# kdu3613/Multimodal_GAR

Measured on AMD Instinct MI355X. Metric: clips/sec (fwd+bwd) at 32 actors x 16k pts x 15 frames, higher is better.
Workload: dtype f32; 1 GPU; c3: 8 clips x 15 frames x 32 actors x 16384 pts, 720x1280 RGB, fp32 fwd+bwd+Adam, LiDAR route pointnet2, GAT on; global_clips=8, clips_per_gpu=8, parallelism=dp1, launch=hip_graph, geometry=in step, gradient_exchange=none, trainable_params=29692332

## Files before the change

include/mgar_ops.h:

```cpp
#ifndef MGAR_OPS_H
#define MGAR_OPS_H

#ifdef __cplusplus
extern "C" {
#endif

#define MGAR_OK 0
#define MGAR_EINVAL (-1)
#define MGAR_ELAUNCH (-2)
#define MGAR_EUNSUPPORTED (-3)

#define MGAR_MAX_NSAMPLE 128
#define MGAR_ABI_VERSION 22

int mgar_abi_version(void);
const char *mgar_last_error(void);

int mgar_ktimer_enable(int on);
int mgar_ktimer_count(void);
const char *mgar_ktimer_name(int id);
int mgar_ktimer_read(int id, double *total_ms, long long *launches, double *total_bytes, double *total_flops,
                     int reset);
int mgar_ktimer_add_flops(int id, double flops);
int mgar_ktimer_add_bytes(int id, double bytes);
// ... 209 lines not shown
                                  int Cout, const float *in_mean, const float *in_invstd, const float *in_gamma,
                                  const float *in_beta, int in_relu, float *y, float *out_stats, void *stream);

int mgar_bn_act_maxpool_bwd_reduce(const float *dpool, long long sb, long long sc, long long sm, const float *pooled,
                                   const unsigned char *arg, const float *x, const float *xarg, int B, int C, int M,
                                   int nsample, const float *mean, const float *invstd, int relu, float *workspace,
                                   float *dgamma, float *dbeta, float *coef, float *dmask, void *stream);
int mgar_pointwise_conv_fwd_maxgrad(const float *x4, int B, int Cin, int M, int nsample, const float *w, int w_row_stride,
                                    int w_col_stride, int Cout, const float *mean, const float *invstd, const float *gamma,
                                    const float *coef, const unsigned char *arg, const float *dmask, float *y, void *stream);
int mgar_pointwise_conv_dw_maxgrad(const float *x, const float *x4, int B, int Cin, int Cout, int M, int nsample,
                                   const float *in_mean, const float *in_invstd, const float *in_gamma,
                                   const float *in_beta, int in_relu, const float *mean, const float *invstd,
                                   const float *gamma, const float *coef, const unsigned char *arg, const float *dmask,
                                   float *workspace, float *dw, void *stream);

int mgar_pointwise_conv_maxpool_eval_fwd(const float *x, int B, int Cin, int M, int nsample, const float *w,
                                         int w_row_stride, int w_col_stride, int Cout, const float *in_mean,
                                         const float *in_invstd, const float *in_gamma, const float *in_beta, int in_relu,
                                         const float *out_scale, const float *out_shift, int out_relu, float *pooled,
                                         void *stream);

int mgar_pointwise_mfma_bf16_fwd(const void *x, int B, int Cin, int P, const float *w, int w_row_stride, int w_col_stride,
                                 int Cout, const float *in_mean, const float *in_invstd, const float *in_gamma,
                                 const float *in_beta, int in_relu, void *y, void *stream);

int mgar_pointwise_wide_bf16_fwd(const void *x, int B, int Cin, int P, const float *w, int w_ld, int Cout,
                                 const float *in_mean, const float *in_invstd, const float *in_gamma, const float *in_beta,
                                 int in_relu, const float *out_scale, const float *out_shift, int out_relu, void *y,
                                 long long y_batch_stride, void *stream);
// ... 230 lines not shown
```

multimodal_gar_amd/bn_ops.py:

```python
import os

import torch
import torch.nn as nn
from torch.autograd import Function
from torch.autograd.function import once_differentiable

from . import _lib as L


def _u8ptr(t):
    return L.dev_ptr(t, torch.uint8)


def _workspace(x, b, c, p):
    return torch.empty((L.raw("mgar_bn_workspace_floats", b, c, p),), dtype=torch.float32, device=x.device)


_PAYLOADS = (torch.float32, torch.bfloat16)


def _f32(t):
    return t if t is None or t.dtype == torch.float32 else t.float()


# ... 130 lines not shown
        ctx.relu = relu
        return y

    @staticmethod
    @once_differentiable
    def backward(ctx, gy):
        x3, gamma, beta, mean, invstd, w = ctx.saved_tensors
        b, c, p = x3.shape
        cout = w.shape[0]
        gy = gy.contiguous()
        st = L.stream_of(x3)
        ga = torch.empty_like(x3)
        L.call("mgar_pointwise_conv_fwd", L.fptr(gy), b, cout, p, L.fptr(w), 1, c, c, None, None, None, None, 0,
               L.fptr(ga), st)
        dgamma, dbeta = torch.empty_like(gamma), torch.empty_like(gamma)
        if FUSED_DW_BN_REDUCE and ctx.needs_input_grad[6]:
            dw = torch.empty_like(w)
            coef = torch.empty((2 * c,), dtype=torch.float32, device=x3.device)
            wsd = torch.empty((max(1, L.raw("mgar_pointwise_dw_bnbwd_workspace_floats", b, c, cout, p)),), dtype=torch.float32,
                              device=x3.device)
            L.call("mgar_pointwise_conv_dw_bnbwd", L.fptr(x3), L.fptr(gy), L.fptr(w), b, c, cout, p, L.fptr(mean), L.fptr(invstd),
                   L.fptr(gamma), L.fptr(beta), int(ctx.relu), L.fptr(wsd), L.fptr(dw), L.fptr(dgamma), L.fptr(dbeta), L.fptr(coef), st)
            dx = torch.empty((b, p, c) if ctx.rowmajor else (b, c, p), dtype=torch.float32, device=x3.device)
            L.call("mgar_bn_act_bwd_apply", L.fptr(ga), L.fptr(x3), b, c, p, L.fptr(mean), L.fptr(invstd), L.fptr(gamma), L.fptr(beta),
                   int(ctx.relu), L.fptr(coef), int(ctx.rowmajor), L.fptr(dx), st)
            return (dx.permute(0, 2, 1) if ctx.rowmajor else dx), dgamma, dbeta, None, None, None, dw, None, None
        dw = None
        if ctx.needs_input_grad[6]:
            dw = torch.empty_like(w)
            wsd = torch.empty((max(1, L.raw("mgar_pointwise_dw_workspace_floats", b, c, cout, p)),), dtype=torch.float32,
                              device=x3.device)
# ... 47 lines not shown
        coef2 = torch.empty((2 * ck,), dtype=torch.float32, device=dev)
        dmask = torch.empty((b, ck, m), dtype=torch.float32, device=dev)
        ws2 = _workspace(x4, b, ck, p)
        if dpool.dtype == torch.float32 and dpool.dim() == 3 and not dpool.is_contiguous() \
                and (b == 1 or dpool.stride(0) >= 0) and min(dpool.stride(1), dpool.stride(2)) >= 1:
            dp, strides = dpool, (dpool.stride(0) if b > 1 else 0, dpool.stride(1), dpool.stride(2))
        else:
            dp, strides = dpool.contiguous().float(), (0, -1, 1)
        L.call("mgar_bn_act_maxpool_bwd_reduce", dp.data_ptr(), strides[0], strides[1], strides[2], L.fptr(out), _u8ptr(arg),
               L.fptr(x4), L.fptr(xarg) if xarg is not None else None, b, ck, m, ns, L.fptr(mean2), L.fptr(invstd2),
               int(ctx.relu2), L.fptr(ws2), L.fptr(dgamma2), L.fptr(dbeta2), L.fptr(coef2), L.fptr(dmask), st)
        ga = torch.empty_like(x3)
        L.call("mgar_pointwise_conv_fwd_maxgrad", L.fptr(x4), b, ck, m, ns, L.fptr(w), 1, c, c, L.fptr(mean2), L.fptr(invstd2),
               L.fptr(gamma2), L.fptr(coef2), _u8ptr(arg), L.fptr(dmask), L.fptr(ga), st)
        dw = None
        if ctx.needs_input_grad[6]:
            dw = torch.empty_like(w)
            wsd = torch.empty((max(1, L.raw("mgar_pointwise_dw_workspace_floats", b, c, ck, p)),), dtype=torch.float32, device=dev)
            L.call("mgar_pointwise_conv_dw_maxgrad", L.fptr(x3), L.fptr(x4), b, c, ck, m, ns, L.fptr(mean), L.fptr(invstd),
                   L.fptr(gamma), L.fptr(beta), int(ctx.relu), L.fptr(mean2), L.fptr(invstd2), L.fptr(gamma2), L.fptr(coef2),
                   _u8ptr(arg), L.fptr(dmask), L.fptr(wsd), L.fptr(dw), st)
        dgamma, dbeta = torch.empty_like(gamma), torch.empty_like(gamma)
        ws = _workspace(x3, b, c, p)
        if ctx.rowmajor:
            dx = _bwd_rowmajor(ga, x3, mean, invstd, gamma, beta, ctx.relu, ws, dgamma, dbeta)
        else:
            dx = torch.empty_like(x3)
            L.call("mgar_bn_act_bwd", L.fptr(ga), L.fptr(x3), b, c, p, L.fptr(mean), L.fptr(invstd), L.fptr(gamma),
                   L.fptr(beta), int(ctx.relu), L.fptr(ws), L.fptr(dgamma), L.fptr(dbeta), L.fptr(dx), st)
        return dx, dgamma, dbeta, None, None, None, dw, dgamma2, dbeta2, None, None, None, None, None


class _PlainConv(Function):

    @staticmethod
    def forward(ctx, x3, w, out_stats=None):
        b, c, p = x3.shape
# ... 41 lines not shown
        return None
    c, cout = x.shape[1], conv.out_channels
    x3 = x.contiguous().flatten(2)
    if c > PLAIN_CONV_MAX_IN or cout > PLAIN_CONV_MAX_OUT or x3.shape[2] % 4 != 0 or x3.shape[0] * x3.shape[2] < (1 << 16):
        return None
    needs_grad = torch.is_grad_enabled() and (x.requires_grad or conv.weight.requires_grad)
    if bf16_mfma and mlp_bf16_mfma_plan(x3, cout, needs_grad, None, PLAIN_CONV_MAX_IN, PLAIN_CONV_MAX_OUT):
        y = _conv_bf16_mfma(x3, _f32(conv.weight.detach()).view(cout, c), None, None, None, None, False)
        y = y.view(x.shape[0], cout, *x.shape[2:])
        return (y, None) if want_out_stats else y
    out_stats = stats_partial_buffer(x3, cout, x3.shape[0] * x3.shape[2]) if want_out_stats and x3.shape[2] % STATS_TILE == 0 else None
    y = _PlainConv.apply(x3, _f32(conv.weight).view(cout, c), out_stats).view(x.shape[0], cout, *x.shape[2:])
    return (y, out_stats) if want_out_stats else y


FUSED_DW_BN_REDUCE = False
FUSED_CONV_MAX_CHANNELS = 64


FUSED_STATS_MAX_CHANNELS = 32


MLP_BF16_MFMA = os.environ.get("MGAR_MLP_BF16_MFMA", "1") != "0"


def mlp_bf16_mfma_plan(x, cout, needs_grad, bn=None, max_in=FUSED_CONV_MAX_CHANNELS, max_out=FUSED_CONV_MAX_CHANNELS):
    if not (MLP_BF16_MFMA and x.dtype == torch.bfloat16 and x.is_cuda and len(x.shape) >= 3) or needs_grad:
        return False
    if bn is not None and not bn.training:
        return False
    c, p = x.shape[1], 1
# ... 504 lines not shown
```

multimodal_gar_amd/csrc/pointwise_dw.hip:

```cpp
#include "common.hpp"

namespace mgar {

typedef float __attribute__((ext_vector_type(16))) f32x16;

constexpr int DW_TP = 128;
constexpr int DW_LD = DW_TP + 1;

struct DwAct {
    const float *mean, *invstd, *gamma, *beta;
    int relu;
    int pair;
};

struct DwGrad {
    const float *mean, *invstd, *gamma;
    const float *coef;
    const unsigned char *arg;
    const float *d;
    int M, ns;
};

template <int OB, int IB, bool GRAD = false>
__global__ __launch_bounds__(256) void pointwise_dw_kernel(const float *__restrict__ x, const float *__restrict__ dy, int B, int Cin,
                                                           int Cout, int P, DwAct act, float *__restrict__ partial, DwGrad g) {
    extern __shared__ float lds[];
    constexpr int GR = GRAD ? OB * 32 : 1;
    __shared__ float g_k[GR], g_m0[GR], g_mu[GR], g_is[GR], g_m1[GR];
    __shared__ float act_sc[IB * 32], act_sh[IB * 32], act_mu[IB * 32];
    __shared__ float act_is[IB * 32];
    float *sy = lds;
    float *sx = lds + OB * 32 * DW_LD;
    const int o_base = blockIdx.y * OB * 32, i_base = blockIdx.z * IB * 32;
    const bool has_act = act.mean != nullptr;
    const bool pair = act.pair != 0;
    const int CinV = pair ? 2 * Cin : Cin;
    if constexpr (GRAD) {
        for (int r = threadIdx.x; r < OB * 32; r += 256) {
            const int ch = o_base + r;
            const bool ok = ch < Cout;
            const float is = ok ? g.invstd[ch] : 0.f;
            g_mu[r] = ok ? g.mean[ch] : 0.f;
            g_is[r] = is;
            g_k[r] = ok ? (g.gamma ? g.gamma[ch] : 1.f) * is : 0.f;
            g_m0[r] = ok ? g.coef[2 * ch] : 0.f;
            g_m1[r] = ok ? g.coef[2 * ch + 1] : 0.f;
        }
        if (!has_act) __syncthreads();
    }
    if (has_act) {
        for (int r = threadIdx.x; r < IB * 32; r += 256) {
            const int chv = i_base + r, ch = (pair && chv >= Cin) ? chv - Cin : chv;
            float sc = 1.f, sh = 0.f, mu = 0.f, is = 0.f;
            if (chv < CinV) {
                sc = act.invstd[ch] * (act.gamma ? act.gamma[ch] : 1.f);
                sh = act.beta ? act.beta[ch] : 0.f;
                mu = act.mean[ch];
                is = act.invstd[ch];
            }
            act_sc[r] = sc;
            act_sh[r] = sh;
            act_mu[r] = mu;
            act_is[r] = is;
        }
        __syncthreads();
    }
    auto pair_of = [&](float v, int r, bool kind) {
        const float mu = act_mu[r];
        const bool on = !act.relu || !((v - mu) * act_sc[r] + act_sh[r] <= 0.f);
        return on ? (kind ? (v - mu) * act_is[r] : 1.f) : 0.f;
    };
    const int lane = threadIdx.x & 63, wave = threadIdx.x >> 6;
    const int tiles_per_b = (P + DW_TP - 1) / DW_TP;
    const long long total_tiles = (long long)B * tiles_per_b;
    const bool vec = (P & 3) == 0;

    f32x16 acc[OB][IB];
#pragma unroll
    for (int a = 0; a < OB; ++a)
#pragma unroll
        for (int c = 0; c < IB; ++c)
#pragma unroll
            for (int r = 0; r < 16; ++r) acc[a][c][r] = 0.f;

    constexpr int NV = (OB + IB) * 32 * (DW_TP / 4) / 256;
    float4 pre[NV];
    constexpr int NG = GRAD ? OB * 4 : 1;
    float pre_d[NG];
    int pre_a[NG], pre_s0 = 0;
    auto fetch = [&](long long tile) {
        const int b = (int)(tile / tiles_per_b);
        const int p0 = (int)(tile - (long long)b * tiles_per_b) * DW_TP;
        if constexpr (GRAD) {
            const int p = p0 + (threadIdx.x & 31) * 4;
            const int m = (int)((unsigned)p / (unsigned)g.ns);
            pre_s0 = p - m * g.ns;
#pragma unroll
            for (int u = 0; u < NG; ++u) {
                const int ch = o_base + (threadIdx.x >> 5) + 8 * u;
                const bool ok = ch < Cout && p < P;
                const size_t go = ((size_t)b * Cout + ch) * g.M + m;
                pre_d[u] = ok ? g.d[go] : 0.f;
                pre_a[u] = ok ? (int)g.arg[go] : 0;
            }
        }
#pragma unroll
        for (int u = 0; u < NV; ++u) {
            const int e = threadIdx.x + u * 256;
            const int row = e / (DW_TP / 4), c4 = (e - row * (DW_TP / 4)) * 4;
            const bool is_y = row < OB * 32;
            const int chv = is_y ? o_base + row : i_base + row - OB * 32;
            const int ch = (!is_y && pair && chv >= Cin) ? chv - Cin : chv;
            const int cmax = is_y ? Cout : Cin;
            pre[u] = (chv < (is_y ? Cout : CinV) && p0 + c4 < P)
                         ? *reinterpret_cast<const float4 *>((is_y ? dy : x) + ((size_t)b * cmax + ch) * P + p0 + c4)
                         : make_float4(0.f, 0.f, 0.f, 0.f);
        }
    };
    if (vec && (long long)blockIdx.x < total_tiles) fetch(blockIdx.x);

    for (long long tile = blockIdx.x; tile < total_tiles; tile += gridDim.x) {
        const int b = (int)(tile / tiles_per_b);
        const int p0 = (int)(tile - (long long)b * tiles_per_b) * DW_TP;
        if (vec) {
#pragma unroll
            for (int u = 0; u < NV; ++u) {
                const int e = threadIdx.x + u * 256;
                const int row = e / (DW_TP / 4), c4 = (e - row * (DW_TP / 4)) * 4;
                const bool is_y = row < OB * 32;
                const int ch = is_y ? o_base + row : i_base + row - OB * 32;
                float4 v = pre[u];
                if constexpr (GRAD) {
                    if (u < NG && ch < Cout && p0 + c4 < P) {
                        const float k = g_k[row], m0 = g_m0[row], mu = g_mu[row], is = g_is[row], m1 = g_m1[row];
                        const float d = pre_d[u < NG ? u : 0];
                        const int sa = pre_a[u < NG ? u : 0] - pre_s0;
                        v.x = k * ((sa == 0 ? d : 0.f) - m0 - (v.x - mu) * is * m1);
                        v.y = k * ((sa == 1 ? d : 0.f) - m0 - (v.y - mu) * is * m1);
                        v.z = k * ((sa == 2 ? d : 0.f) - m0 - (v.z - mu) * is * m1);
                        v.w = k * ((sa == 3 ? d : 0.f) - m0 - (v.w - mu) * is * m1);
                    }
                }
                if (has_act && !is_y && ch < CinV && p0 + c4 < P) {
                    const int r = row - OB * 32;
                    if (pair) {
                        const bool kind = ch >= Cin;
                        v.x = pair_of(v.x, r, kind); v.y = pair_of(v.y, r, kind); v.z = pair_of(v.z, r, kind); v.w = pair_of(v.w, r, kind);
                    } else {
                        const float sc = act_sc[r], sh = act_sh[r], mu = act_mu[r];
                        v.x = (v.x - mu) * sc + sh; v.y = (v.y - mu) * sc + sh; v.z = (v.z - mu) * sc + sh; v.w = (v.w - mu) * sc + sh;
                        if (act.relu) { v.x = relu_nan(v.x); v.y = relu_nan(v.y); v.z = relu_nan(v.z); v.w = relu_nan(v.w); }
                    }
                }
                float *d = lds + row * DW_LD + c4;
                d[0] = v.x; d[1] = v.y; d[2] = v.z; d[3] = v.w;
            }
        } else {
            for (int e = threadIdx.x; e < (OB + IB) * 32 * DW_TP; e += 256) {
                const int row = e / DW_TP, cc = e - row * DW_TP;
                const bool is_y = row < OB * 32;
                const int chv = is_y ? o_base + row : i_base + row - OB * 32;
                const int ch = (!is_y && pair && chv >= Cin) ? chv - Cin : chv;
                const int cmax = is_y ? Cout : Cin;
                float v = 0.f;
                if (chv < (is_y ? Cout : CinV) && p0 + cc < P) {
                    v = (is_y ? dy : x)[((size_t)b * cmax + ch) * P + p0 + cc];
                    if (has_act && !is_y) {
                        if (pair) {
                            v = pair_of(v, row - OB * 32, chv >= Cin);
                        } else {
                            v = (v - act_mu[row - OB * 32]) * act_sc[row - OB * 32] + act_sh[row - OB * 32];
                            if (act.relu) v = relu_nan(v);
                        }
                    }
                }
                lds[row * DW_LD + cc] = v;
            }
        }
        __syncthreads();
        if (vec && tile + gridDim.x < total_tiles) fetch(tile + gridDim.x);
        const int colw = wave * 32 + (lane >> 5);
#pragma unroll 4
        for (int ks = 0; ks < 16; ++ks) {
            const int cc = colw + 2 * ks;
            float af[OB], bf[IB];
#pragma unroll
            for (int a = 0; a < OB; ++a) af[a] = sy[(a * 32 + (lane & 31)) * DW_LD + cc];
#pragma unroll
            for (int c = 0; c < IB; ++c) bf[c] = sx[(c * 32 + (lane & 31)) * DW_LD + cc];
#pragma unroll
            for (int a = 0; a < OB; ++a)
#pragma unroll
                for (int c = 0; c < IB; ++c)
                    acc[a][c] = __builtin_amdgcn_mfma_f32_32x32x2f32(af[a], bf[c], acc[a][c], 0, 0, 0);
        }
        __syncthreads();
    }
    if (wave > 0) {
#pragma unroll
        for (int a = 0; a < OB; ++a)
#pragma unroll
            for (int c = 0; c < IB; ++c)
#pragma unroll
                for (int r = 0; r < 16; ++r) lds[(((wave - 1) * OB * IB + a * IB + c) * 16 + r) * 64 + lane] = acc[a][c][r];
    }
    __syncthreads();
    if (wave > 0) return;
#pragma unroll
    for (int a = 0; a < OB; ++a)
#pragma unroll
        for (int c = 0; c < IB; ++c)
#pragma unroll
            for (int r = 0; r < 16; ++r) {
                float v = acc[a][c][r];
#pragma unroll
                for (int w = 0; w < 3; ++w) v += lds[((w * OB * IB + a * IB + c) * 16 + r) * 64 + lane];
                const int o = o_base + a * 32 + (r & 3) + 8 * (r >> 2) + 4 * (lane >> 5);
                const int i = i_base + c * 32 + (lane & 31);
                if (o < Cout && i < CinV) partial[((size_t)blockIdx.x * Cout + o) * CinV + i] = v;
            }
}

constexpr int DWR_SLICES = 16;
__global__ __launch_bounds__(64 * DWR_SLICES) void pointwise_dw_reduce_kernel(const float *__restrict__ partial, int gx, int n_out,
                                                                              float *__restrict__ dw) {
    __shared__ float part[DWR_SLICES][64];
    const int e = blockIdx.x * 64 + (threadIdx.x & 63), slice = threadIdx.x >> 6;
    const int per = (gx + DWR_SLICES - 1) / DWR_SLICES, g0 = min(slice * per, gx), g1 = min(g0 + per, gx);
    float s = 0.f;
    if (e < n_out) {
        int g = g0;
        for (; g + 8 <= g1; g += 8) {
            float v[8];
#pragma unroll
// ... 34 lines not shown
}

static int dw_grid_x(int B, int Cin, int Cout, int P, int ob, int ib) {
    const long long tiles = (long long)B * ((P + DW_TP - 1) / DW_TP);
    const int gy = ceil_div(Cout, ob * 32), gz = ceil_div(Cin, ib * 32);
    long long gx = 2048 / (gy * gz);
    if (gx > (tiles + 3) / 4) gx = (tiles + 3) / 4;
    if (gx < 1) gx = 1;
    return (int)gx;
}
static void dw_blocks(int Cin, int Cout, int &ob, int &ib) {
    ob = Cout <= 32 ? 1 : 2;
    ib = Cin <= 32 ? 1 : (Cin <= 64 ? 2 : 4);
}

template <int OB, int IB, bool GRAD = false>
static void launch_dw(const float *x, const float *dy, int B, int Cin, int Cout, int P, const DwAct &act, float *partial,
                      hipStream_t st, const DwGrad &g = DwGrad{}) {
    static bool attr_set = false;
    const int lds = (OB + IB) * 32 * DW_LD * (int)sizeof(float);
    if (!attr_set) {
        (void)hipFuncSetAttribute((const void *)pointwise_dw_kernel<OB, IB, GRAD>, hipFuncAttributeMaxDynamicSharedMemorySize, lds);
        attr_set = true;
    }
    const int CinV = act.pair ? 2 * Cin : Cin;
    const int gy = ceil_div(Cout, OB * 32), gz = ceil_div(CinV, IB * 32);
    const int gx = dw_grid_x(B, CinV, Cout, P, OB, IB);
    hipLaunchKernelGGL((pointwise_dw_kernel<OB, IB, GRAD>), dim3((unsigned)gx, gy, gz), dim3(256), lds, st, x, dy, B, Cin, Cout, P, act, partial, g);
}

}

using namespace mgar;

MGAR_API int mgar_pointwise_dw_workspace_floats(int B, int Cin, int Cout, int P) {
    if (B <= 0 || Cin <= 0 || Cout <= 0 || P <= 0) return 0;
    int ob, ib;
    dw_blocks(Cin, Cout, ob, ib);
    return dw_grid_x(B, Cin, Cout, P, ob, ib) * Cout * Cin;
}

MGAR_API int mgar_pointwise_conv_dw_act(const float *x, const float *dy, int B, int Cin,
                                        int Cout, int P, const float *in_mean,
// ... 1 lines not shown
                                        const float *in_beta, int in_relu,
                                        float *workspace, float *dw, void *stream) {
    MGAR_REQUIRE(B >= 0 && Cin >= 0 && Cout >= 0 && P >= 0, "pointwise_conv_dw: negative size");
    if (Cin == 0 || Cout == 0) return MGAR_OK;
    MGAR_REQUIRE(dw, "pointwise_conv_dw: null pointer");
    MGAR_REQUIRE(in_mean == nullptr || in_invstd != nullptr, "pointwise_conv_dw: in_mean without in_invstd");
    hipStream_t st = (hipStream_t)stream;
    if ((long long)B * P == 0) {
        (void)hipMemsetAsync(dw, 0, sizeof(float) * Cout * Cin, st);
        return check_launch("pointwise_conv_dw: memset failed");
    }
    MGAR_REQUIRE(x && dy && workspace, "pointwise_conv_dw: null pointer");
    const DwAct act{in_mean, in_invstd, in_gamma, in_beta, in_relu, 0};
    int ob, ib;
    dw_blocks(Cin, Cout, ob, ib);
    {
    KtScope kt(KT_POINTWISE_DW, st, 4.0 * (double)B * P * (Cin + Cout), 2.0 * (double)B * P * Cin * Cout);
    if (ob == 1 && ib == 1) launch_dw<1, 1>(x, dy, B, Cin, Cout, P, act, workspace, st);
    else if (ob == 1 && ib == 2) launch_dw<1, 2>(x, dy, B, Cin, Cout, P, act, workspace, st);
    else if (ob == 1 && ib == 4) launch_dw<1, 4>(x, dy, B, Cin, Cout, P, act, workspace, st);
    else if (ob == 2 && ib == 1) launch_dw<2, 1>(x, dy, B, Cin, Cout, P, act, workspace, st);
    else if (ob == 2 && ib == 2) launch_dw<2, 2>(x, dy, B, Cin, Cout, P, act, workspace, st);
    else launch_dw<2, 4>(x, dy, B, Cin, Cout, P, act, workspace, st);
    }
    const int gx = dw_grid_x(B, Cin, Cout, P, ob, ib), n_out = Cout * Cin;
    hipLaunchKernelGGL(pointwise_dw_reduce_kernel, dim3(ceil_div(n_out, 64)), dim3(64 * DWR_SLICES), 0, st, workspace, gx, n_out, dw);
    return check_launch("pointwise_conv_dw: launch failed");
}

MGAR_API int mgar_pointwise_conv_dw(const float *x, const float *dy, int B, int Cin,
                                    int Cout, int P, float *workspace, float *dw,
                                    void *stream) {
    return mgar_pointwise_conv_dw_act(x, dy, B, Cin, Cout, P, nullptr, nullptr, nullptr, nullptr, 0, workspace, dw, stream);
}

MGAR_API int mgar_pointwise_conv_dw_maxgrad(const float *x, const float *x4, int B, int Cin, int Cout, int M, int nsample,
                                            const float *in_mean, const float *in_invstd, const float *in_gamma,
                                            const float *in_beta, int in_relu, const float *mean, const float *invstd,
                                            const float *gamma, const float *coef, const unsigned char *arg, const float *dmask,
                                            float *workspace, float *dw, void *stream) {
// ... 6 lines not shown
        set_error("pointwise_conv_dw_maxgrad: needs Cin <= 64, Cout <= 64 and nsample % 4 == 0 (write the gradient with "
                  "mgar_bn_act_maxpool_bwd otherwise)");
        return MGAR_EUNSUPPORTED;
    }
    hipStream_t st = (hipStream_t)stream;
    if ((long long)B * M == 0) {
        (void)hipMemsetAsync(dw, 0, sizeof(float) * Cout * Cin, st);
        return check_launch("pointwise_conv_dw_maxgrad: memset failed");
    }
    MGAR_REQUIRE(x && x4 && workspace && mean && invstd && coef && arg && dmask, "pointwise_conv_dw_maxgrad: null pointer");
    const int P = M * nsample;
    const DwAct act{in_mean, in_invstd, in_gamma, in_beta, in_relu, 0};
    const DwGrad g{mean, invstd, gamma, coef, arg, dmask, M, nsample};
    int ob, ib;
    dw_blocks(Cin, Cout, ob, ib);
    {
    KtScope kt(KT_POINTWISE_DW, st, 4.0 * (double)B * P * (Cin + Cout) + 5.0 * (double)B * Cout * M, 2.0 * (double)B * P * Cin * Cout);
    if (ob == 1 && ib == 1) launch_dw<1, 1, true>(x, x4, B, Cin, Cout, P, act, workspace, st, g);
    else if (ob == 1) launch_dw<1, 2, true>(x, x4, B, Cin, Cout, P, act, workspace, st, g);
    else if (ib == 1) launch_dw<2, 1, true>(x, x4, B, Cin, Cout, P, act, workspace, st, g);
    else launch_dw<2, 2, true>(x, x4, B, Cin, Cout, P, act, workspace, st, g);
    }
    const int gx = dw_grid_x(B, Cin, Cout, P, ob, ib), n_out = Cout * Cin;
    hipLaunchKernelGGL(pointwise_dw_reduce_kernel, dim3(ceil_div(n_out, 64)), dim3(64 * DWR_SLICES), 0, st, workspace, gx, n_out, dw);
    return check_launch("pointwise_conv_dw_maxgrad: launch failed");
}

MGAR_API int mgar_pointwise_dw_bnbwd_workspace_floats(int B, int Cin, int Cout, int P) {
    if (B <= 0 || Cin <= 0 || Cout <= 0 || P <= 0) return 0;
    int ob, ib;
    dw_blocks(2 * Cin, Cout, ob, ib);
    return dw_grid_x(B, 2 * Cin, Cout, P, ob, ib) * Cout * 2 * Cin + Cout * 2 * Cin;
}
MGAR_API int mgar_pointwise_conv_dw_bnbwd(const float *x, const float *dy, const float *w, int B,
                                          int Cin, int Cout, int P, const float *in_mean,
                                          const float *in_invstd, const float *in_gamma,
                                          const float *in_beta, int in_relu, float *workspace,
                                          float *dw, float *dgamma, float *dbeta, float *coef,
                                          void *stream) {
    MGAR_REQUIRE(B >= 0 && Cin >= 1 && Cout >= 1 && P >= 0, "pointwise_conv_dw_bnbwd: bad sizes");
    if (Cin > 64 || Cout > 64) {
        set_error("pointwise_conv_dw_bnbwd: Cin <= 64 and Cout <= 64");
        return MGAR_EUNSUPPORTED;
    }
    MGAR_REQUIRE((long long)B * P > 0, "pointwise_conv_dw_bnbwd: empty input");
    MGAR_REQUIRE(x && dy && w && in_mean && in_invstd && workspace && coef, "pointwise_conv_dw_bnbwd: null pointer");
    hipStream_t st = (hipStream_t)stream;
    const DwAct act{in_mean, in_invstd, in_gamma, in_beta, in_relu, 1};
    int ob, ib;
    dw_blocks(2 * Cin, Cout, ob, ib);
    const int gx = dw_grid_x(B, 2 * Cin, Cout, P, ob, ib), n_out = Cout * 2 * Cin;
    float *ab = workspace + (size_t)gx * n_out;
    {
        KtScope kt(KT_POINTWISE_DW, st, 4.0 * (double)B * P * (Cin + Cout), 4.0 * (double)B * P * Cin * Cout);
        if (ob == 1 && ib == 1) launch_dw<1, 1>(x, dy, B, Cin, Cout, P, act, workspace, st);
        else if (ob == 1 && ib == 2) launch_dw<1, 2>(x, dy, B, Cin, Cout, P, act, workspace, st);
        else if (ob == 1 && ib == 4) launch_dw<1, 4>(x, dy, B, Cin, Cout, P, act, workspace, st);
        else if (ob == 2 && ib == 1) launch_dw<2, 1>(x, dy, B, Cin, Cout, P, act, workspace, st);
        else if (ob == 2 && ib == 2) launch_dw<2, 2>(x, dy, B, Cin, Cout, P, act, workspace, st);
        else launch_dw<2, 4>(x, dy, B, Cin, Cout, P, act, workspace, st);
    }
    hipLaunchKernelGGL(pointwise_dw_reduce_kernel, dim3(ceil_div(n_out, 64)), dim3(64 * DWR_SLICES), 0, st, workspace, gx, n_out, ab);
    hipLaunchKernelGGL(pointwise_dw_pair_finalize_kernel, dim3(ceil_div(Cin, 64)), dim3(64), 0, st, ab, w, Cin, Cout, (double)B * P, in_gamma,
                       in_beta, dw, dgamma, dbeta, coef);
    return check_launch("pointwise_conv_dw_bnbwd: launch failed");
}
```

Before: 46.35 clips/sec.

## Restructure pointwise dw kernel into per-wave swizzled LDS tiles, add maxgrad fused BN path

```diff
diff --git a/include/mgar_ops.h b/include/mgar_ops.h
--- a/include/mgar_ops.h
+++ b/include/mgar_ops.h
@@ -247,6 +247,11 @@
                                    const float *in_beta, int in_relu, const float *mean, const float *invstd,
                                    const float *gamma, const float *coef, const unsigned char *arg, const float *dmask,
                                    float *workspace, float *dw, void *stream);
+int mgar_maxgrad_conv_dw_bnbwd(const float *x, const float *x4, const float *w, int B, int Cin, int Cout, int M,
+                                         int nsample, const float *in_mean, const float *in_invstd, const float *in_gamma,
+                                         const float *in_beta, int in_relu, const float *mean, const float *invstd,
+                                         const float *gamma, const float *coef2, const unsigned char *arg, const float *dmask,
+                                         float *workspace, float *dw, float *dgamma, float *dbeta, float *coef, void *stream);
 
 int mgar_pointwise_conv_maxpool_eval_fwd(const float *x, int B, int Cin, int M, int nsample, const float *w,
                                          int w_row_stride, int w_col_stride, int Cout, const float *in_mean,
diff --git a/multimodal_gar_amd/bn_ops.py b/multimodal_gar_amd/bn_ops.py
--- a/multimodal_gar_amd/bn_ops.py
+++ b/multimodal_gar_amd/bn_ops.py
@@ -168,7 +168,7 @@
         L.call("mgar_pointwise_conv_fwd", L.fptr(gy), b, cout, p, L.fptr(w), 1, c, c, None, None, None, None, 0,
                L.fptr(ga), st)
         dgamma, dbeta = torch.empty_like(gamma), torch.empty_like(gamma)
-        if FUSED_DW_BN_REDUCE and ctx.needs_input_grad[6]:
+        if ctx.needs_input_grad[6] and fused_dw_bn_plan(c, cout, b * p):
             dw = torch.empty_like(w)
             coef = torch.empty((2 * c,), dtype=torch.float32, device=x3.device)
             wsd = torch.empty((max(1, L.raw("mgar_pointwise_dw_bnbwd_workspace_floats", b, c, cout, p)),), dtype=torch.float32,
@@ -246,13 +246,26 @@
         L.call("mgar_pointwise_conv_fwd_maxgrad", L.fptr(x4), b, ck, m, ns, L.fptr(w), 1, c, c, L.fptr(mean2), L.fptr(invstd2),
                L.fptr(gamma2), L.fptr(coef2), _u8ptr(arg), L.fptr(dmask), L.fptr(ga), st)
         dw = None
+        dgamma, dbeta = torch.empty_like(gamma), torch.empty_like(gamma)
+        if ctx.needs_input_grad[6] and fused_dw_bn_plan(c, ck, b * p):
+            dw = torch.empty_like(w)
+            coef = torch.empty((2 * c,), dtype=torch.float32, device=dev)
+            wsd = torch.empty((max(1, L.raw("mgar_pointwise_dw_bnbwd_workspace_floats", b, c, ck, p)),), dtype=torch.float32, device=dev)
+            L.call("mgar_maxgrad_conv_dw_bnbwd", L.fptr(x3), L.fptr(x4), L.fptr(w), b, c, ck, m, ns, L.fptr(mean),
+                   L.fptr(invstd), L.fptr(gamma), L.fptr(beta), int(ctx.relu), L.fptr(mean2), L.fptr(invstd2), L.fptr(gamma2),
+                   L.fptr(coef2), _u8ptr(arg), L.fptr(dmask), L.fptr(wsd), L.fptr(dw), L.fptr(dgamma), L.fptr(dbeta), L.fptr(coef), st)
+            dx = torch.empty((b, p, c) if ctx.rowmajor else (b, c, p), dtype=torch.float32, device=dev)
+            L.call("mgar_bn_act_bwd_apply", L.fptr(ga), L.fptr(x3), b, c, p, L.fptr(mean), L.fptr(invstd), L.fptr(gamma), L.fptr(beta),
+                   int(ctx.relu), L.fptr(coef), int(ctx.rowmajor), L.fptr(dx), st)
+            if ctx.rowmajor:
+                dx = dx.permute(0, 2, 1)
+            return dx, dgamma, dbeta, None, None, None, dw, dgamma2, dbeta2, None, None, None, None, None
         if ctx.needs_input_grad[6]:
             dw = torch.empty_like(w)
             wsd = torch.empty((max(1, L.raw("mgar_pointwise_dw_workspace_floats", b, c, ck, p)),), dtype=torch.float32, device=dev)
             L.call("mgar_pointwise_conv_dw_maxgrad", L.fptr(x3), L.fptr(x4), b, c, ck, m, ns, L.fptr(mean), L.fptr(invstd),
                    L.fptr(gamma), L.fptr(beta), int(ctx.relu), L.fptr(mean2), L.fptr(invstd2), L.fptr(gamma2), L.fptr(coef2),
                    _u8ptr(arg), L.fptr(dmask), L.fptr(wsd), L.fptr(dw), st)
-        dgamma, dbeta = torch.empty_like(gamma), torch.empty_like(gamma)
         ws = _workspace(x3, b, c, p)
         if ctx.rowmajor:
             dx = _bwd_rowmajor(ga, x3, mean, invstd, gamma, beta, ctx.relu, ws, dgamma, dbeta)
@@ -324,7 +337,21 @@
     return (y, out_stats) if want_out_stats else y
 
 
-FUSED_DW_BN_REDUCE = False
+FUSED_DW_BN_REDUCE = os.environ.get("MGAR_FUSED_DW_BN_REDUCE", "0") == "1"
+FUSED_DW_BN_MIN_COLUMNS = 1 << 16
+FUSED_DW_BN_MIN_CIN = 17
+_FUSED_DW_BN_BLOCKS = {(1, 1): True, (1, 2): True, (2, 1): True, (2, 2): False}
+
+
+def fused_dw_bn_plan(cin, cout, columns, switch=None):
+    on = FUSED_DW_BN_REDUCE if switch is None else switch
+    if not on or cin < 1 or cout < 1 or cin > FUSED_CONV_MAX_CHANNELS or cout > FUSED_CONV_MAX_CHANNELS:
+        return False
+    if columns < FUSED_DW_BN_MIN_COLUMNS or cin < FUSED_DW_BN_MIN_CIN:
+        return False
+    return _FUSED_DW_BN_BLOCKS[((cin + 31) // 32, (cout + 31) // 32)]
+
+
 FUSED_CONV_MAX_CHANNELS = 64
 
 
diff --git a/multimodal_gar_amd/csrc/pointwise_dw.hip b/multimodal_gar_amd/csrc/pointwise_dw.hip
--- a/multimodal_gar_amd/csrc/pointwise_dw.hip
+++ b/multimodal_gar_amd/csrc/pointwise_dw.hip
@@ -5,7 +5,7 @@
 typedef float __attribute__((ext_vector_type(16))) f32x16;
 
 constexpr int DW_TP = 128;
-constexpr int DW_LD = DW_TP + 1;
+constexpr int DW_WC = 32;
 
 struct DwAct {
     const float *mean, *invstd, *gamma, *beta;
@@ -21,20 +21,26 @@
     int M, ns;
 };
 
-template <int OB, int IB, bool GRAD = false>
-__global__ __launch_bounds__(256) void pointwise_dw_kernel(const float *__restrict__ x, const float *__restrict__ dy, int B, int Cin,
-                                                           int Cout, int P, DwAct act, float *__restrict__ partial, DwGrad g) {
-    extern __shared__ float lds[];
+__device__ __forceinline__ void dw_wave_sync() {
+    __builtin_amdgcn_fence(__ATOMIC_RELEASE, "wavefront");
+    __builtin_amdgcn_wave_barrier();
+    __builtin_amdgcn_fence(__ATOMIC_ACQUIRE, "wavefront");
+}
+
+template <int OB, int IB, bool GRAD, bool PAIR>
+__global__ __launch_bounds__(256, (OB + IB <= 4 && OB * IB * (PAIR ? 2 : 1) <= 4 ? 2 : 1)) void pointwise_dw_kernel(
+    const float *__restrict__ x, const float *__restrict__ dy, int B, int Cin, int Cout, int P, DwAct act, float *__restrict__ partial,
+    DwGrad g) {
+    extern __shared__ __attribute__((aligned(16))) float lds[];
+    constexpr int IBV = PAIR ? 2 * IB : IB;
+    constexpr int ROWS = (OB + IB) * 32;
     constexpr int GR = GRAD ? OB * 32 : 1;
     __shared__ float g_k[GR], g_m0[GR], g_mu[GR], g_is[GR], g_m1[GR];
     __shared__ float act_sc[IB * 32], act_sh[IB * 32], act_mu[IB * 32];
     __shared__ float act_is[IB * 32];
-    float *sy = lds;
-    float *sx = lds + OB * 32 * DW_LD;
     const int o_base = blockIdx.y * OB * 32, i_base = blockIdx.z * IB * 32;
     const bool has_act = act.mean != nullptr;
-    const bool pair = act.pair != 0;
-    const int CinV = pair ? 2 * Cin : Cin;
+    const int CinV = PAIR ? 2 * Cin : Cin;
     if constexpr (GRAD) {
         for (int r = threadIdx.x; r < OB * 32; r += 256) {
             const int ch = o_base + r;
@@ -50,9 +56,9 @@
     }
     if (has_act) {
         for (int r = threadIdx.x; r < IB * 32; r += 256) {
-            const int chv = i_base + r, ch = (pair && chv >= Cin) ? chv - Cin : chv;
+            const int ch = i_base + r;
             float sc = 1.f, sh = 0.f, mu = 0.f, is = 0.f;
-            if (chv < CinV) {
+            if (ch < Cin) {
                 sc = act.invstd[ch] * (act.gamma ? act.gamma[ch] : 1.f);
                 sh = act.beta ? act.beta[ch] : 0.f;
                 mu = act.mean[ch];
@@ -65,40 +71,57 @@
         }
         __syncthreads();
     }
-    auto pair_of = [&](float v, int r, bool kind) {
-        const float mu = act_mu[r];
-        const bool on = !act.relu || !((v - mu) * act_sc[r] + act_sh[r] <= 0.f);
-        return on ? (kind ? (v - mu) * act_is[r] : 1.f) : 0.f;
-    };
     const int lane = threadIdx.x & 63, wave = threadIdx.x >> 6;
     const int tiles_per_b = (P + DW_TP - 1) / DW_TP;
     const long long total_tiles = (long long)B * tiles_per_b;
     const bool vec = (P & 3) == 0;
-
-    f32x16 acc[OB][IB];
+    float *wl = lds + wave * ROWS * DW_WC;
+
+    const int lq = lane & 7, lg = lane >> 3;
+    const int lrow = 8 * (lg & 1) + (lg >> 1);
+    auto row_of = [&](int u) { return 16 * (u >> 1) + 4 * (u & 1) + lrow; };
+    auto lds_pos = [](int row, int pi) { return row * DW_WC + ((((pi >> 2) ^ (row >> 1)) & 7) << 2) + (pi & 3); };
+    const int mr = lane & 31, mh = lane >> 5;
+    int rd_off[4];
+#pragma unroll
+    for (int j = 0; j < 4; ++j) rd_off[j] = lds_pos(mr, (mh * 4 + j) * 4);
+
+    float p_mu[IB], p_sc[IB], p_sh[IB], p_is[IB];
+    if constexpr (PAIR) {
+#pragma unroll
+        for (int c = 0; c < IB; ++c) {
+            p_mu[c] = act_mu[c * 32 + mr];
+            p_sc[c] = act_sc[c * 32 + mr];
+            p_sh[c] = act_sh[c * 32 + mr];
+            p_is[c] = act_is[c * 32 + mr];
+        }
+    }
+
+    f32x16 acc[OB][IBV];
 #pragma unroll
     for (int a = 0; a < OB; ++a)
 #pragma unroll
-        for (int c = 0; c < IB; ++c)
+        for (int c = 0; c < IBV; ++c)
 #pragma unroll
             for (int r = 0; r < 16; ++r) acc[a][c][r] = 0.f;
 
-    constexpr int NV = (OB + IB) * 32 * (DW_TP / 4) / 256;
+    constexpr int NV = (OB + IB) * 4;
     float4 pre[NV];
     constexpr int NG = GRAD ? OB * 4 : 1;
     float pre_d[NG];
     int pre_a[NG], pre_s0 = 0;
+    bool pre_ok = false;
     auto fetch = [&](long long tile) {
         const int b = (int)(tile / tiles_per_b);
-        const int p0 = (int)(tile - (long long)b * tiles_per_b) * DW_TP;
+        const int p = (int)(tile - (long long)b * tiles_per_b) * DW_TP + wave * DW_WC + lq * 4;
+        pre_ok = p < P;
         if constexpr (GRAD) {
-            const int p = p0 + (threadIdx.x & 31) * 4;
             const int m = (int)((unsigned)p / (unsigned)g.ns);
             pre_s0 = p - m * g.ns;
 #pragma unroll
             for (int u = 0; u < NG; ++u) {
-                const int ch = o_base + (threadIdx.x >> 5) + 8 * u;
-                const bool ok = ch < Cout && p < P;
+                const int ch = o_base + row_of(u);
+                const bool ok = ch < Cout && pre_ok;
                 const size_t go = ((size_t)b * Cout + ch) * g.M + m;
                 pre_d[u] = ok ? g.d[go] : 0.f;
                 pre_a[u] = ok ? (int)g.arg[go] : 0;
@@ -106,32 +129,27 @@
         }
 #pragma unroll
         for (int u = 0; u < NV; ++u) {
-            const int e = threadIdx.x + u * 256;
-            const int row = e / (DW_TP / 4), c4 = (e - row * (DW_TP / 4)) * 4;
-            const bool is_y = row < OB * 32;
-            const int chv = is_y ? o_base + row : i_base + row - OB * 32;
-            const int ch = (!is_y && pair && chv >= Cin) ? chv - Cin : chv;
+            const bool is_y = u < OB * 4;
+            const int ch = is_y ? o_base + row_of(u) : i_base + row_of(u) - OB * 32;
             const int cmax = is_y ? Cout : Cin;
-            pre[u] = (chv < (is_y ? Cout : CinV) && p0 + c4 < P)
-                         ? *reinterpret_cast<const float4 *>((is_y ? dy : x) + ((size_t)b * cmax + ch) * P + p0 + c4)
-                         : make_float4(0.f, 0.f, 0.f, 0.f);
+            pre[u] = (ch < cmax && pre_ok) ? *reinterpret_cast<const float4 *>((is_y ? dy : x) + ((size_t)b * cmax + ch) * P + p)
+                                           : make_float4(0.f, 0.f, 0.f, 0.f);
         }
     };
     if (vec && (long long)blockIdx.x < total_tiles) fetch(blockIdx.x);
 
     for (long long tile = blockIdx.x; tile < total_tiles; tile += gridDim.x) {
         const int b = (int)(tile / tiles_per_b);
-        const int p0 = (int)(tile - (long long)b * tiles_per_b) * DW_TP;
+        const int pw = (int)(tile - (long long)b * tiles_per_b) * DW_TP + wave * DW_WC;
         if (vec) {
 #pragma unroll
             for (int u = 0; u < NV; ++u) {
-                const int e = threadIdx.x + u * 256;
-                const int row = e / (DW_TP / 4), c4 = (e - row * (DW_TP / 4)) * 4;
-                const bool is_y = row < OB * 32;
+                const bool is_y = u < OB * 4;
+                const int row = row_of(u);
                 const int ch = is_y ? o_base + row : i_base + row - OB * 32;
                 float4 v = pre[u];
                 if constexpr (GRAD) {
-                    if (u < NG && ch < Cout && p0 + c4 < P) {
+                    if (u < NG && ch < Cout && pre_ok) {
                         const float k = g_k[row], m0 = g_m0[row], mu = g_mu[row], is = g_is[row], m1 = g_m1[row];
                         const float d = pre_d[u < NG ? u : 0];
                         const int sa = pre_a[u < NG ? u : 0] - pre_s0;
@@ -141,83 +159,101 @@
                         v.w = k * ((sa == 3 ? d : 0.f) - m0 - (v.w - mu) * is * m1);
                     }
                 }
-                if (has_act && !is_y && ch < CinV && p0 + c4 < P) {
+                if (!PAIR && has_act && !is_y && ch < Cin && pre_ok) {
                     const int r = row - OB * 32;
-                    if (pair) {
-                        const bool kind = ch >= Cin;
-                        v.x = pair_of(v.x, r, kind); v.y = pair_of(v.y, r, kind); v.z = pair_of(v.z, r, kind); v.w = pair_of(v.w, r, kind);
-                    } else {
-                        const float sc = act_sc[r], sh = act_sh[r], mu = act_mu[r];
-                        v.x = (v.x - mu) * sc + sh; v.y = (v.y - mu) * sc + sh; v.z = (v.z - mu) * sc + sh; v.w = (v.w - mu) * sc + sh;
-                        if (act.relu) { v.x = relu_nan(v.x); v.y = relu_nan(v.y); v.z = relu_nan(v.z); v.w = relu_nan(v.w); }
+                    const float sc = act_sc[r], sh = act_sh[r], mu = act_mu[r];
+                    v.x = (v.x - mu) * sc + sh; v.y = (v.y - mu) * sc + sh; v.z = (v.z - mu) * sc + sh; v.w = (v.w - mu) * sc + sh;
+                    if (act.relu) { v.x = relu_nan(v.x); v.y = relu_nan(v.y); v.z = relu_nan(v.z); v.w = relu_nan(v.w); }
+                }
+                *reinterpret_cast<float2 *>(wl + lds_pos(row, 2 * lq)) = make_float2(v.x, v.z);
+                *reinterpret_cast<float2 *>(wl + lds_pos(row, 16 + 2 * lq)) = make_float2(v.y, v.w);
+            }
+        } else {
+            for (int e = lane; e < ROWS * DW_WC; e += 64) {
+                const int row = e / DW_WC, cc = e - row * DW_WC;
+                const bool is_y = row < OB * 32;
+                const int ch = is_y ? o_base + row : i_base + row - OB * 32;
+                const int cmax = is_y ? Cout : Cin;
+                float v = 0.f;
+                if (ch < cmax && pw + cc < P) {
+                    v = (is_y ? dy : x)[((size_t)b * cmax + ch) * P + pw + cc];
+                    if (!PAIR && has_act && !is_y) {
+                        v = (v - act_mu[row - OB * 32]) * act_sc[row - OB * 32] + act_sh[row - OB * 32];
+                        if (act.relu) v = relu_nan(v);
                     }
                 }
-                float *d = lds + row * DW_LD + c4;
-                d[0] = v.x; d[1] = v.y; d[2] = v.z; d[3] = v.w;
-            }
-        } else {
-            for (int e = threadIdx.x; e < (OB + IB) * 32 * DW_TP; e += 256) {
-                const int row = e / DW_TP, cc = e - row * DW_TP;
-                const bool is_y = row < OB * 32;
-                const int chv = is_y ? o_base + row : i_base + row - OB * 32;
-                const int ch = (!is_y && pair && chv >= Cin) ? chv - Cin : chv;
-                const int cmax = is_y ? Cout : Cin;
-                float v = 0.f;
-                if (chv < (is_y ? Cout : CinV) && p0 + cc < P) {
-                    v = (is_y ? dy : x)[((size_t)b * cmax + ch) * P + p0 + cc];
-                    if (has_act && !is_y) {
-                        if (pair) {
-                            v = pair_of(v, row - OB * 32, chv >= Cin);
-                        } else {
-                            v = (v - act_mu[row - OB * 32]) * act_sc[row - OB * 32] + act_sh[row - OB * 32];
-                            if (act.relu) v = relu_nan(v);
-                        }
+                wl[lds_pos(row, (cc & 1) * 16 + (cc >> 1))] = v;
+            }
+        }
+        dw_wave_sync();
+        if (vec && tile + gridDim.x < total_tiles) fetch(tile + gridDim.x);
+        const int nvalid = P - pw;
+#pragma unroll
+        for (int j = 0; j < 4; ++j) {
+            float4 af[OB], bf[IB];
+#pragma unroll
+            for (int a = 0; a < OB; ++a) af[a] = *reinterpret_cast<const float4 *>(wl + a * 32 * DW_WC + rd_off[j]);
+#pragma unroll
+            for (int c = 0; c < IB; ++c) bf[c] = *reinterpret_cast<const float4 *>(wl + (OB + c) * 32 * DW_WC + rd_off[j]);
+#pragma unroll
+            for (int t = 0; t < 4; ++t) {
+                float av[OB], bv[IBV];
+#pragma unroll
+                for (int a = 0; a < OB; ++a) av[a] = t == 0 ? af[a].x : t == 1 ? af[a].y : t == 2 ? af[a].z : af[a].w;
+#pragma unroll
+                for (int c = 0; c < IB; ++c) {
+                    const float v = t == 0 ? bf[c].x : t == 1 ? bf[c].y : t == 2 ? bf[c].z : bf[c].w;
+                    if constexpr (PAIR) {
+                        const bool inside = 2 * (4 * j + t) + mh < nvalid;
+                        const bool on = inside && (!act.relu || !((v - p_mu[c]) * p_sc[c] + p_sh[c] <= 0.f));
+                        bv[c] = on ? 1.f : 0.f;
+                        bv[IB + c] = on ? (v - p_mu[c]) * p_is[c] : 0.f;
+                    } else {
+                        bv[c] = v;
                     }
                 }
-                lds[row * DW_LD + cc] = v;
-            }
+#pragma unroll
+                for (int a = 0; a < OB; ++a)
+#pragma unroll
+                    for (int c = 0; c < IBV; ++c)
+                        acc[a][c] = __builtin_amdgcn_mfma_f32_32x32x2f32(av[a], bv[c], acc[a][c], 0, 0, 0);
+            }
+        }
+        dw_wave_sync();
+    }
+    __syncthreads();
+#pragma unroll 1
+    for (int w = 1; w < 4; ++w) {
+        if (wave == w) {
+#pragma unroll
+            for (int a = 0; a < OB; ++a)
+#pragma unroll
+                for (int c = 0; c < IBV; ++c)
+#pragma unroll
+                    for (int r = 0; r < 16; ++r) lds[((a * IBV + c) * 16 + r) * 64 + lane] = acc[a][c][r];
         }
         __syncthreads();
-        if (vec && tile + gridDim.x < total_tiles) fetch(tile + gridDim.x);
-        const int colw = wave * 32 + (lane >> 5);
-#pragma unroll 4
-        for (int ks = 0; ks < 16; ++ks) {
-            const int cc = colw + 2 * ks;
-            float af[OB], bf[IB];
-#pragma unroll
-            for (int a = 0; a < OB; ++a) af[a] = sy[(a * 32 + (lane & 31)) * DW_LD + cc];
-#pragma unroll
-            for (int c = 0; c < IB; ++c) bf[c] = sx[(c * 32 + (lane & 31)) * DW_LD + cc];
+        if (wave == 0) {
 #pragma unroll
             for (int a = 0; a < OB; ++a)
 #pragma unroll
-                for (int c = 0; c < IB; ++c)
-                    acc[a][c] = __builtin_amdgcn_mfma_f32_32x32x2f32(af[a], bf[c], acc[a][c], 0, 0, 0);
+                for (int c = 0; c < IBV; ++c)
+#pragma unroll
+                    for (int r = 0; r < 16; ++r) acc[a][c][r] += lds[((a * IBV + c) * 16 + r) * 64 + lane];
         }
         __syncthreads();
     }
-    if (wave > 0) {
-#pragma unroll
-        for (int a = 0; a < OB; ++a)
-#pragma unroll
-            for (int c = 0; c < IB; ++c)
-#pragma unroll
-                for (int r = 0; r < 16; ++r) lds[(((wave - 1) * OB * IB + a * IB + c) * 16 + r) * 64 + lane] = acc[a][c][r];
-    }
-    __syncthreads();
     if (wave > 0) return;
 #pragma unroll
     for (int a = 0; a < OB; ++a)
 #pragma unroll
-        for (int c = 0; c < IB; ++c)
+        for (int c = 0; c < IBV; ++c)
 #pragma unroll
             for (int r = 0; r < 16; ++r) {
-                float v = acc[a][c][r];
-#pragma unroll
-                for (int w = 0; w < 3; ++w) v += lds[((w * OB * IB + a * IB + c) * 16 + r) * 64 + lane];
                 const int o = o_base + a * 32 + (r & 3) + 8 * (r >> 2) + 4 * (lane >> 5);
-                const int i = i_base + c * 32 + (lane & 31);
-                if (o < Cout && i < CinV) partial[((size_t)blockIdx.x * Cout + o) * CinV + i] = v;
+                const int i = i_base + (PAIR ? c % IB : c) * 32 + (lane & 31);
+                const int iv = (PAIR && c >= IB) ? Cin + i : i;
+                if (o < Cout && i < Cin) partial[((size_t)blockIdx.x * Cout + o) * CinV + iv] = acc[a][c][r];
             }
 }
 
@@ -282,19 +318,39 @@
     ib = Cin <= 32 ? 1 : (Cin <= 64 ? 2 : 4);
 }
 
-template <int OB, int IB, bool GRAD = false>
-static void launch_dw(const float *x, const float *dy, int B, int Cin, int Cout, int P, const DwAct &act, float *partial,
-                      hipStream_t st, const DwGrad &g = DwGrad{}) {
+template <int OB, int IB, bool GRAD, bool PAIR>
+static void launch_dw(const float *x, const float *dy, int B, int Cin, int Cout, int P, const DwAct &act, float *partial, int gx,
+                      hipStream_t st, const DwGrad &g) {
     static bool attr_set = false;
-    const int lds = (OB + IB) * 32 * DW_LD * (int)sizeof(float);
+    const int lds = 4 * (OB + IB) * 32 * DW_WC * (int)sizeof(float);
     if (!attr_set) {
-        (void)hipFuncSetAttribute((const void *)pointwise_dw_kernel<OB, IB, GRAD>, hipFuncAttributeMaxDynamicSharedMemorySize, lds);
+        (void)hipFuncSetAttribute((const void *)pointwise_dw_kernel<OB, IB, GRAD, PAIR>, hipFuncAttributeMaxDynamicSharedMemorySize, lds);
         attr_set = true;
     }
-    const int CinV = act.pair ? 2 * Cin : Cin;
-    const int gy = ceil_div(Cout, OB * 32), gz = ceil_div(CinV, IB * 32);
-    const int gx = dw_grid_x(B, CinV, Cout, P, OB, IB);
-    hipLaunchKernelGGL((pointwise_dw_kernel<OB, IB, GRAD>), dim3((unsigned)gx, gy, gz), dim3(256), lds, st, x, dy, B, Cin, Cout, P, act, partial, g);
+    const int gy = ceil_div(Cout, OB * 32), gz = ceil_div(Cin, IB * 32);
+    hipLaunchKernelGGL((pointwise_dw_kernel<OB, IB, GRAD, PAIR>), dim3((unsigned)gx, gy, gz), dim3(256), lds, st, x, dy, B, Cin, Cout, P, act,
+                       partial, g);
+}
+
+template <bool GRAD, bool PAIR>
+static void dispatch_dw(const float *x, const float *dy, int B, int Cin, int Cout, int P, const DwAct &act, float *partial, int gx,
+                        hipStream_t st, const DwGrad &g = DwGrad{}) {
+    int ob, ib;
+    dw_blocks(Cin, Cout, ob, ib);
+    if (ob == 1 && ib == 1) launch_dw<1, 1, GRAD, PAIR>(x, dy, B, Cin, Cout, P, act, partial, gx, st, g);
+    else if (ob == 1 && ib == 2) launch_dw<1, 2, GRAD, PAIR>(x, dy, B, Cin, Cout, P, act, partial, gx, st, g);
+    else if (ob == 2 && ib == 1) launch_dw<2, 1, GRAD, PAIR>(x, dy, B, Cin, Cout, P, act, partial, gx, st, g);
+    else if (ob == 2 && ib == 2) launch_dw<2, 2, GRAD, PAIR>(x, dy, B, Cin, Cout, P, act, partial, gx, st, g);
+    else if constexpr (!GRAD && !PAIR) {
+        if (ob == 1) launch_dw<1, 4, false, false>(x, dy, B, Cin, Cout, P, act, partial, gx, st, g);
+        else launch_dw<2, 4, false, false>(x, dy, B, Cin, Cout, P, act, partial, gx, st, g);
+    }
+}
+
+static int dw_pair_grid_x(int B, int Cin, int Cout, int P) {
+    int ob, ib;
+    dw_blocks(2 * Cin, Cout, ob, ib);
+    return dw_grid_x(B, 2 * Cin, Cout, P, ob, ib);
 }
 
 }
@@ -326,16 +382,11 @@
     const DwAct act{in_mean, in_invstd, in_gamma, in_beta, in_relu, 0};
     int ob, ib;
     dw_blocks(Cin, Cout, ob, ib);
+    const int gx = dw_grid_x(B, Cin, Cout, P, ob, ib), n_out = Cout * Cin;
     {
     KtScope kt(KT_POINTWISE_DW, st, 4.0 * (double)B * P * (Cin + Cout), 2.0 * (double)B * P * Cin * Cout);
-    if (ob == 1 && ib == 1) launch_dw<1, 1>(x, dy, B, Cin, Cout, P, act, workspace, st);
-    else if (ob == 1 && ib == 2) launch_dw<1, 2>(x, dy, B, Cin, Cout, P, act, workspace, st);
-    else if (ob == 1 && ib == 4) launch_dw<1, 4>(x, dy, B, Cin, Cout, P, act, workspace, st);
-    else if (ob == 2 && ib == 1) launch_dw<2, 1>(x, dy, B, Cin, Cout, P, act, workspace, st);
-    else if (ob == 2 && ib == 2) launch_dw<2, 2>(x, dy, B, Cin, Cout, P, act, workspace, st);
-    else launch_dw<2, 4>(x, dy, B, Cin, Cout, P, act, workspace, st);
-    }
-    const int gx = dw_grid_x(B, Cin, Cout, P, ob, ib), n_out = Cout * Cin;
+    dispatch_dw<false, false>(x, dy, B, Cin, Cout, P, act, workspace, gx, st);
+    }
     hipLaunchKernelGGL(pointwise_dw_reduce_kernel, dim3(ceil_div(n_out, 64)), dim3(64 * DWR_SLICES), 0, st, workspace, gx, n_out, dw);
     return check_launch("pointwise_conv_dw: launch failed");
 }
@@ -372,23 +423,18 @@
     const DwGrad g{mean, invstd, gamma, coef, arg, dmask, M, nsample};
     int ob, ib;
     dw_blocks(Cin, Cout, ob, ib);
+    const int gx = dw_grid_x(B, Cin, Cout, P, ob, ib), n_out = Cout * Cin;
     {
     KtScope kt(KT_POINTWISE_DW, st, 4.0 * (double)B * P * (Cin + Cout) + 5.0 * (double)B * Cout * M, 2.0 * (double)B * P * Cin * Cout);
-    if (ob == 1 && ib == 1) launch_dw<1, 1, true>(x, x4, B, Cin, Cout, P, act, workspace, st, g);
-    else if (ob == 1) launch_dw<1, 2, true>(x, x4, B, Cin, Cout, P, act, workspace, st, g);
-    else if (ib == 1) launch_dw<2, 1, true>(x, x4, B, Cin, Cout, P, act, workspace, st, g);
-    else launch_dw<2, 2, true>(x, x4, B, Cin, Cout, P, act, workspace, st, g);
-    }
-    const int gx = dw_grid_x(B, Cin, Cout, P, ob, ib), n_out = Cout * Cin;
+    dispatch_dw<true, false>(x, x4, B, Cin, Cout, P, act, workspace, gx, st, g);
+    }
     hipLaunchKernelGGL(pointwise_dw_reduce_kernel, dim3(ceil_div(n_out, 64)), dim3(64 * DWR_SLICES), 0, st, workspace, gx, n_out, dw);
     return check_launch("pointwise_conv_dw_maxgrad: launch failed");
 }
 
 MGAR_API int mgar_pointwise_dw_bnbwd_workspace_floats(int B, int Cin, int Cout, int P) {
     if (B <= 0 || Cin <= 0 || Cout <= 0 || P <= 0) return 0;
-    int ob, ib;
-    dw_blocks(2 * Cin, Cout, ob, ib);
-    return dw_grid_x(B, 2 * Cin, Cout, P, ob, ib) * Cout * 2 * Cin + Cout * 2 * Cin;
+    return dw_pair_grid_x(B, Cin, Cout, P) * Cout * 2 * Cin + Cout * 2 * Cin;
 }
 MGAR_API int mgar_pointwise_conv_dw_bnbwd(const float *x, const float *dy, const float *w, int B,
                                           int Cin, int Cout, int P, const float *in_mean,
@@ -405,21 +451,45 @@
     MGAR_REQUIRE(x && dy && w && in_mean && in_invstd && workspace && coef, "pointwise_conv_dw_bnbwd: null pointer");
     hipStream_t st = (hipStream_t)stream;
     const DwAct act{in_mean, in_invstd, in_gamma, in_beta, in_relu, 1};
-    int ob, ib;
-    dw_blocks(2 * Cin, Cout, ob, ib);
-    const int gx = dw_grid_x(B, 2 * Cin, Cout, P, ob, ib), n_out = Cout * 2 * Cin;
+    const int gx = dw_pair_grid_x(B, Cin, Cout, P), n_out = Cout * 2 * Cin;
     float *ab = workspace + (size_t)gx * n_out;
     {
         KtScope kt(KT_POINTWISE_DW, st, 4.0 * (double)B * P * (Cin + Cout), 4.0 * (double)B * P * Cin * Cout);
-        if (ob == 1 && ib == 1) launch_dw<1, 1>(x, dy, B, Cin, Cout, P, act, workspace, st);
-        else if (ob == 1 && ib == 2) launch_dw<1, 2>(x, dy, B, Cin, Cout, P, act, workspace, st);
-        else if (ob == 1 && ib == 4) launch_dw<1, 4>(x, dy, B, Cin, Cout, P, act, workspace, st);
-        else if (ob == 2 && ib == 1) launch_dw<2, 1>(x, dy, B, Cin, Cout, P, act, workspace, st);
-        else if (ob == 2 && ib == 2) launch_dw<2, 2>(x, dy, B, Cin, Cout, P, act, workspace, st);
-        else launch_dw<2, 4>(x, dy, B, Cin, Cout, P, act, workspace, st);
+        dispatch_dw<false, true>(x, dy, B, Cin, Cout, P, act, workspace, gx, st);
     }
     hipLaunchKernelGGL(pointwise_dw_reduce_kernel, dim3(ceil_div(n_out, 64)), dim3(64 * DWR_SLICES), 0, st, workspace, gx, n_out, ab);
     hipLaunchKernelGGL(pointwise_dw_pair_finalize_kernel, dim3(ceil_div(Cin, 64)), dim3(64), 0, st, ab, w, Cin, Cout, (double)B * P, in_gamma,
                        in_beta, dw, dgamma, dbeta, coef);
     return check_launch("pointwise_conv_dw_bnbwd: launch failed");
 }
+
+MGAR_API int mgar_maxgrad_conv_dw_bnbwd(const float *x, const float *x4, const float *w, int B, int Cin, int Cout, int M,
+                                                  int nsample, const float *in_mean, const float *in_invstd,
+                                                  const float *in_gamma, const float *in_beta, int in_relu, const float *mean,
+                                                  const float *invstd, const float *gamma, const float *coef2,
+                                                  const unsigned char *arg, const float *dmask, float *workspace, float *dw,
+                                                  float *dgamma, float *dbeta, float *coef, void *stream) {
+    MGAR_REQUIRE(B >= 0 && Cin >= 1 && Cout >= 1 && M >= 0 && nsample >= 1 && nsample <= 255, "maxgrad_conv_dw_bnbwd: bad sizes");
+    MGAR_REQUIRE((long long)M * nsample <= 2147483647LL - DW_TP, "maxgrad_conv_dw_bnbwd: M * nsample too large");
+    if (Cin > 64 || Cout > 64 || (nsample & 3) != 0) {
+        set_error("maxgrad_conv_dw_bnbwd: needs Cin <= 64, Cout <= 64 and nsample % 4 == 0");
+        return MGAR_EUNSUPPORTED;
+    }
+    MGAR_REQUIRE((long long)B * M > 0, "maxgrad_conv_dw_bnbwd: empty input");
+    MGAR_REQUIRE(x && x4 && w && in_mean && in_invstd && workspace && coef && mean && invstd && coef2 && arg && dmask,
+                 "maxgrad_conv_dw_bnbwd: null pointer");
+    hipStream_t st = (hipStream_t)stream;
+    const int P = M * nsample;
+    const DwAct act{in_mean, in_invstd, in_gamma, in_beta, in_relu, 1};
+    const DwGrad g{mean, invstd, gamma, coef2, arg, dmask, M, nsample};
+    const int gx = dw_pair_grid_x(B, Cin, Cout, P), n_out = Cout * 2 * Cin;
+    float *ab = workspace + (size_t)gx * n_out;
+    {
+        KtScope kt(KT_POINTWISE_DW, st, 4.0 * (double)B * P * (Cin + Cout) + 5.0 * (double)B * Cout * M, 4.0 * (double)B * P * Cin * Cout);
+        dispatch_dw<true, true>(x, x4, B, Cin, Cout, P, act, workspace, gx, st, g);
+    }
+    hipLaunchKernelGGL(pointwise_dw_reduce_kernel, dim3(ceil_div(n_out, 64)), dim3(64 * DWR_SLICES), 0, st, workspace, gx, n_out, ab);
+    hipLaunchKernelGGL(pointwise_dw_pair_finalize_kernel, dim3(ceil_div(Cin, 64)), dim3(64), 0, st, ab, w, Cin, Cout, (double)B * P, in_gamma,
+                       in_beta, dw, dgamma, dbeta, coef);
+    return check_launch("maxgrad_conv_dw_bnbwd: launch failed");
+}
```

Measured after the change: 46.23 clips/sec. About the same (-0.3%).
